# neuromodulation/PyPARRM

Hardware: NVIDIA B200
Metric: filter_data channel-samples/sec (higher is better)
Workload: dtype f64

## Files before the change

### pyparrm_b200/csrc/filter_comb_e.cuh

```cuda
#pragma once

#ifdef __CUDACC_RTC__
typedef signed char int8_t;
typedef int int32_t;
typedef unsigned int uint32_t;
typedef long long int64_t;
typedef unsigned long long uint64_t;
typedef unsigned long long uintptr_t;
#else
#include <stdint.h>
#endif

#ifndef PE_D
#define PE_T double
#define PE_D 200
#define PE_NK 2
#define PE_M0 20
#define PE_M1 10
#define PE_NB0 7
#define PE_NB1 2
#define PE_OFF0 -1969, -1954, -1923, -1877, -1846, -1831, -1800
#define PE_OFF1 -1908, 108
#define PE_NPLUS 1
#define PE_PLUS -2000
#define PE_NMINUS 0
#define PE_MINUS 0
#define PE_CENTRE -1
#define PE_U 10
#define PE_PF 2
#define PE_NTAPS 160
#define PE_WLO -2000
#define PE_WHI 2000
#define PE_BACK 108
#define PE_FWD 2000
#define PE_CTAS 2
#endif
#ifndef PE_VARIANT
#define PE_VARIANT 0
#endif

namespace parrm_e {

typedef PE_T T;
typedef double T2;
constexpr int D = PE_D;
constexpr int NK = PE_NK;
constexpr int M0 = PE_M0;
constexpr int M1 = PE_M1;
constexpr int NB0 = PE_NB0;
constexpr int NB1 = PE_NB1;
constexpr int NPLUS = PE_NPLUS;
constexpr int NMINUS = PE_NMINUS;
constexpr int CENTRE = PE_CENTRE;
constexpr int U = PE_U;
constexpr int PF = PE_PF;
constexpr int NTAPS = PE_NTAPS;
constexpr int WLO = PE_WLO;
constexpr int WHI = PE_WHI;
constexpr int BACK = PE_BACK;
constexpr int FWD = PE_FWD;
constexpr int ES = int(sizeof(T));
constexpr int VEC = 16 / ES;
constexpr int CH = U * D;
constexpr int HB = (BACK + CH - 1) / CH;
constexpr int HF = (FWD + CH - 1) / CH;
constexpr int MIR = HB + HF;
constexpr int Q = HB + HF + 1 + PF;
constexpr int GPB = (M0 + U - 1) / U;
constexpr int B = GPB * U;
constexpr int NPG = GPB;
constexpr int NW = (D + 31) / 32;
constexpr int NT = NW * 32 + 32;
constexpr int BAR_BYTES = ((2 * Q * 8 + 127) / 128) * 128;
constexpr int SMEM_BYTES = BAR_BYTES + (Q + MIR) * CH * ES;
static_assert((CH * ES) % 16 == 0, "chunk must be a whole number of 16-byte units");
static_assert(M0 >= M1 && M0 >= 1, "box lengths ordered");

__host__ __device__ constexpr int off0(int b) {
  constexpr int t[NB0 > 0 ? NB0 : 1] = {PE_OFF0};
  return t[b];
}
__host__ __device__ constexpr int off1(int b) {
  constexpr int t[NB1 > 0 ? NB1 : 1] = {PE_OFF1};
  return t[b];
}
__host__ __device__ constexpr int plus_tap(int i) {
  constexpr int t[NPLUS > 0 ? NPLUS : 1] = {PE_PLUS};
  return t[i];
}
__host__ __device__ constexpr int minus_tap(int i) {
  constexpr int t[NMINUS > 0 ? NMINUS : 1] = {PE_MINUS};
  return t[i];
}

struct Args {
  const T* x;
  T* out;
  const int32_t* taps;
  const int32_t* count;
  const T2* recip;
  int64_t ld_x, x_t0, n_x;
  int64_t ld_out, t0, n_out;
  int64_t n_total;
  int64_t total_groups;
  int32_t groups_per_chan;
  int32_t edge_start;
  int32_t edge_total;
  int32_t pad;
  unsigned long long* timeline;
  T neg_inv_n;
  T t_max;
};

__device__ __forceinline__ uint32_t smem_u32(const void* p) {
  return static_cast<uint32_t>(__cvta_generic_to_shared(p));
}
__device__ __forceinline__ void mbar_init(uint64_t* bar, uint32_t count) {
  asm volatile("mbarrier.init.shared::cta.b64 [%0], %1;" ::"r"(smem_u32(bar)), "r"(count));
}
__device__ __forceinline__ void mbar_expect_tx(uint64_t* bar, uint32_t bytes) {
  asm volatile("mbarrier.arrive.expect_tx.shared::cta.b64 _, [%0], %1;" ::"r"(smem_u32(bar)),
               "r"(bytes)
               : "memory");
}
__device__ __forceinline__ void mbar_arrive(uint64_t* bar) {
  asm volatile("mbarrier.arrive.shared::cta.b64 _, [%0];" ::"r"(smem_u32(bar)) : "memory");
}
__device__ __forceinline__ void mbar_wait(uint32_t bar, uint32_t parity) {
  asm volatile(
      "{\n"
      ".reg .pred p;\n"
      "WAIT_%=:\n"
      "mbarrier.try_wait.parity.shared::cta.b64 p, [%0], %1;\n"
      "@p bra DONE_%=;\n"
      "bra WAIT_%=;\n"
      "DONE_%=:\n"
      "}\n" ::"r"(bar),
      "r"(parity)
      : "memory");
}
__device__ __forceinline__ void bulk_g2s(void* dst_smem, const void* src_gmem, uint32_t bytes,
                                         uint64_t* bar) {
  asm volatile(
      "cp.async.bulk.shared::cluster.global.mbarrier::complete_tx::bytes [%0], [%1], %2, [%3];" ::
          "r"(smem_u32(dst_smem)),
      "l"(src_gmem), "r"(bytes), "r"(smem_u32(bar))
      : "memory");
}

__device__ __forceinline__ int64_t floor_div(int64_t a, int64_t b) {
  int64_t q = a / b;
  return (a % b != 0 && ((a < 0) != (b < 0))) ? q - 1 : q;
}
__device__ __forceinline__ int64_t min64(int64_t a, int64_t b) { return a < b ? a : b; }
__device__ __forceinline__ int64_t max64(int64_t a, int64_t b) { return a > b ? a : b; }

__device__ __forceinline__ T edge_value(const int32_t* __restrict__ count,
                                        const T2* __restrict__ recip, int64_t t, int64_t n_total,
                                        T xc, T tot) {
  const int64_t v1 = min64(max64(t, WLO - 1), WHI);
  const int64_t v2 = min64(max64(t - n_total, WLO - 1), WHI);
  const int n_in = count[v1 - (WLO - 1)] - count[v2 - (WLO - 1)];
  T y = xc - tot * T(recip[n_in]);
  if (n_in == 0) y = T(0);
  return y;
}

__device__ __noinline__ T direct_value(const int32_t* __restrict__ taps,
                                       const T2* __restrict__ recip, int64_t n_total, T t_max,
                                       const T* __restrict__ xrow, int64_t t, int64_t lo_valid,
                                       int64_t hi_valid) {
  T acc = T(0);
  int n_in = 0;
  for (int k = 0; k < NTAPS; ++k) {
    const int64_t g = t - taps[k];
    if (g < 0 || g >= n_total) continue;
    ++n_in;
    if (g >= lo_valid && g < hi_valid) acc += xrow[g];
  }
  if (n_in == 0) return T(0);
  const T y = xrow[t] - acc * T(recip[n_in]);
  return fabs(y) <= t_max ? y : T(0);
}

struct Walk {
  int pb;
  int rslot;
  int fslot;
  uint32_t fphase;
};

__device__ __forceinline__ void group_begin(Walk& w, uint32_t bars) {
  mbar_wait(bars + w.fslot * 8, w.fphase);
  if (++w.fslot == Q) {
    w.fslot = 0;
    w.fphase ^= 1u;
  }
}
__device__ __forceinline__ void group_end(Walk& w, uint32_t bars, int lane, unsigned wmask) {
  __syncwarp(wmask);
  if (lane == 0) {
    asm volatile("mbarrier.arrive.shared::cta.b64 _, [%0];" ::"r"(bars + (Q + w.rslot) * 8)
                 : "memory");
  }
  w.pb += CH * ES;
  if (++w.rslot == Q) {
    w.rslot = 0;
    w.pb -= Q * CH * ES;
  }
}

struct Rings {
  T r0[B];
  T r1[NK > 1 ? B : 1];
  T S0, S1;
};

__device__ __forceinline__ T ring_sum0(const Rings& r, int s) {
  T a = r.r0[s];
#pragma unroll
  for (int i = 1; i < M0; ++i) a += r.r0[(s + B - i) % B];
  return a;
}
__device__ __forceinline__ T ring_sum1(const Rings& r, int s) {
  if (NK < 2) return T(0);
  T a = r.r1[s];
#pragma unroll
  for (int i = 1; i < M1; ++i) a += r.r1[(s + B - i) % B];
  return a;
}

template <bool FAST>
__device__ __forceinline__ int run_block(Rings& r, Walk& w, const Args& a,
                                         const unsigned char* const smem, uint32_t bars,
                                         int lane, unsigned wmask, int c, T* const orow,
                                         int& bad_lo, int& bad_hi, int64_t Tb, int g,
                                         int n_groups) {
  const T neg_inv_n = a.neg_inv_n;
  const T t_max = a.t_max;
  T* const op = orow + Tb + c;
  int done = 0;
#pragma unroll
  for (int gi = 0; gi < GPB; ++gi) {
    if (!FAST && g + gi >= n_groups) break;
    group_begin(w, bars);
    int mode = 1;
    if (!FAST) {
      const int64_t Tn = Tb + int64_t(gi) * CH;
      const bool interior = (Tn - WHI >= 0) && (Tn + CH - WLO <= a.n_total);
      const bool all_out = (Tn >= a.t0) && (Tn + CH <= a.t0 + a.n_out);
      mode = (g + gi < NPG) ? 0 : ((interior && all_out) ? 1 : 2);
    }
    const unsigned char* const p = smem + w.pb;
#pragma unroll
    for (int js = 0; js < U; ++js) {
      const int s = gi * U + js;
      auto ld = [&](int off) {
        return *reinterpret_cast<const T*>(p + (HB * CH + js * D - off) * ES);
      };
      r.S0 -= r.r0[(s + B - M0) % B];
      if (NK > 1) r.S1 -= r.r1[(s + B - M1) % B];
      T e0 = ld(off0(0));
      if (NB0 > 1) {
        T e0b = ld(off0(1));
#pragma unroll
        for (int b = 2; b < NB0; ++b) {
          if (b & 1) e0b += ld(off0(b)); else e0 += ld(off0(b));
        }
        e0 += e0b;
      }
      r.r0[s] = e0;
      r.S0 += e0;
      T tot = r.S0;
      if (NK > 1) {
        T e1 = ld(off1(0));
        if (NB1 > 1) {
          T e1b = ld(off1(1));
#pragma unroll
          for (int b = 2; b < NB1; ++b) {
            if (b & 1) e1b += ld(off1(b)); else e1 += ld(off1(b));
          }
          e1 += e1b;
        }
        r.r1[s] = e1;
        r.S1 += e1;
        tot += r.S1;
      }
      T single = T(0);
      if (NPLUS > 0) {
        single = ld(plus_tap(0));
#pragma unroll
        for (int i = 1; i < NPLUS; ++i) single += ld(plus_tap(i));
      }
#pragma unroll
      for (int i = 0; i < NMINUS; ++i) single -= ld(minus_tap(i));
      const T xc = ld(0);
      if (CENTRE != 0) single = fma(T(CENTRE), xc, single);
      if (NPLUS > 0 || NMINUS > 0 || CENTRE != 0) tot += single;
      if (FAST) {
        T y = fma(tot, neg_inv_n, xc);
        if (__builtin_expect(!(fabs(y) <= t_max), 0)) {
          r.S0 = ring_sum0(r, s);
          r.S1 = ring_sum1(r, s);
          bad_lo = min(bad_lo, g * U + s);
          bad_hi = max(bad_hi, g * U + s);
          y = T(0);
        }
        op[s * D] = y;
      } else if (mode != 0) {
        const int64_t t = Tb + c + int64_t(s) * D;
        if (ES == 4 && mode == 2) {
          r.S0 = ring_sum0(r, s);
          r.S1 = ring_sum1(r, s);
          tot = r.S0;
          if (NK > 1) tot += r.S1;
          if (NPLUS > 0 || NMINUS > 0 || CENTRE != 0) tot += single;
        }
        T y = mode == 1 ? fma(tot, neg_inv_n, xc) : edge_value(a.count, a.recip, t, a.n_total, xc, tot);
        if (__builtin_expect(!(fabs(y) <= t_max), 0)) {
          r.S0 = ring_sum0(r, s);
          r.S1 = ring_sum1(r, s);
          bad_lo = min(bad_lo, g * U + s);
          bad_hi = max(bad_hi, g * U + s);
          y = T(0);
        }
        if (t >= a.t0 && t < a.t0 + a.n_out) op[s * D] = y;
      }
    }
    group_end(w, bars, lane, wmask);
    ++done;
  }
  return done;
}

extern "C" __global__ void __launch_bounds__(NT, PE_CTAS) parrm_filter_comb_e(const Args a) {
  extern __shared__ __align__(128) unsigned char smem_raw[];
  uint64_t* const full = reinterpret_cast<uint64_t*>(smem_raw);
  uint64_t* const empty = full + Q;
  T* const ring = reinterpret_cast<T*>(smem_raw + BAR_BYTES);
  const int tid = threadIdx.x;
  const int lane = tid & 31;
  const bool is_producer = tid >= NW * 32;

  if (tid == 0) {
    for (int s = 0; s < Q; ++s) {
      mbar_init(&full[s], 1);
      mbar_init(&empty[s], NW);
    }
    asm volatile("fence.mbarrier_init.release.cluster;" ::: "memory");
  }
  __syncthreads();

  const int64_t lo_valid = max64(0, a.x_t0);
  const int64_t hi_valid = min64(a.n_total, a.x_t0 + a.n_x);
#if PE_VARIANT & 2
  unsigned long long tl_start = 0, tl_pieces = 0;
  if (tid == 0) asm volatile("mov.u64 %0, %%globaltimer;" : "=l"(tl_start));
#endif
  const int gpc = a.groups_per_chan;
  const int vpc = gpc + a.edge_total;
  const int64_t G_begin = a.total_groups * int64_t(blockIdx.x) / int64_t(gridDim.x);
  const int64_t G_end = a.total_groups * int64_t(blockIdx.x + 1) / int64_t(gridDim.x);
  const uint32_t bars = smem_u32(smem_raw);

  int fslot = 0;
  uint32_t fphase = 0;
  int rslot = 0;

  for (int64_t G = G_begin; G < G_end;) {
    const int64_t chan = G / vpc;
    const int v0 = int(G - chan * vpc);
    const int v1 = int(min64(vpc, v0 + (G_end - G)));
    G += v1 - v0;
    const int s0 = min(max(v0 - a.edge_start, 0), gpc);
    const int s1 = min(max(v1 - a.edge_start, 0), gpc);
    if (s1 <= s0) continue;
    const T* const xrow = a.x + chan * a.ld_x - a.x_t0;
    T* const orow = a.out + chan * a.ld_out - a.t0;
    const int gamma = int((VEC - int((reinterpret_cast<uintptr_t>(xrow) / ES) % VEC)) % VEC);
    const int64_t j_first = floor_div(a.t0 - gamma, CH);
    const int64_t j_last = floor_div(a.t0 + a.n_out - 1 - gamma, CH);
    const int64_t n_first = j_first + s0;
    const int64_t n_end = min64(j_first + s1, j_last + 1);
    if (n_first >= n_end) continue;
#if PE_VARIANT & 2
    ++tl_pieces;
#endif
    const int n_groups = NPG + int(n_end - n_first);
    const int n_chunks = n_groups + HB + HF;
    const int64_t c_first = n_first - NPG - HB;

    if (is_producer) {
      for (int i = 0; i < n_chunks; ++i) {
        const int64_t g0 = gamma + (c_first + i) * int64_t(CH);
        T* const dst = ring + fslot * CH;
        mbar_wait(bars + (Q + fslot) * 8, fphase ^ 1u);
        if (g0 >= lo_valid && g0 + CH <= hi_valid) {
          if (lane == 0) {
            asm volatile("fence.proxy.async.shared::cta;" ::: "memory");
            const bool mirror = fslot < MIR;
            mbar_expect_tx(&full[fslot], uint32_t(CH * ES) * (mirror ? 2u : 1u));
            bulk_g2s(dst, xrow + g0, uint32_t(CH * ES), &full[fslot]);
            if (mirror) bulk_g2s(dst + Q * CH, xrow + g0, uint32_t(CH * ES), &full[fslot]);
          }
        } else {
          for (int e = lane; e < CH; e += 32) {
            const int64_t g = g0 + e;
            const T v = (g >= lo_valid && g < hi_valid) ? xrow[g] : T(0);
            dst[e] = v;
            if (fslot < MIR) dst[Q * CH + e] = v;
          }
          __syncwarp();
          if (lane == 0) mbar_arrive(&full[fslot]);
        }
        if (++fslot == Q) {
          fslot = 0;
          fphase ^= 1u;
        }
      }
      continue;
    }

    if (tid >= D) continue;
    const int c = tid;
    const unsigned wmask = (tid | 31) < D ? 0xffffffffu : ((1u << (D & 31)) - 1u);
    for (int i = 0; i < HB + HF; ++i) {
      mbar_wait(bars + fslot * 8, fphase);
      if (++fslot == Q) {
        fslot = 0;
        fphase ^= 1u;
      }
    }
    Rings r;
#pragma unroll
    for (int s = 0; s < B; ++s) r.r0[s] = T(0);
#pragma unroll
    for (int s = 0; s < (NK > 1 ? B : 1); ++s) r.r1[s] = T(0);
    const int64_t T0 = gamma + (n_first - NPG) * int64_t(CH);
    Walk w;
    w.pb = BAR_BYTES + (rslot * CH + c) * ES;
    w.rslot = rslot;
    w.fslot = fslot;
    w.fphase = fphase;
    int bad_lo = 1 << 30, bad_hi = -1;
    for (int g = 0; g < n_groups;) {
      const int64_t Tb = T0 + int64_t(g) * CH;
      r.S0 = ring_sum0(r, B - 1);
      r.S1 = ring_sum1(r, B - 1);
      const bool fast = g >= NPG && g + GPB <= n_groups && Tb - WHI >= 0 &&
                        Tb + int64_t(B) * D - WLO <= a.n_total && Tb >= a.t0 &&
                        Tb + int64_t(B) * D <= a.t0 + a.n_out;
      if (fast) {
        g += run_block<true>(r, w, a, smem_raw, bars, lane, wmask, c, orow, bad_lo, bad_hi,
                             Tb, g, n_groups);
      } else {
        g += run_block<false>(r, w, a, smem_raw, bars, lane, wmask, c, orow, bad_lo, bad_hi,
                              Tb, g, n_groups);
      }
    }
    rslot = w.rslot;
    fslot = w.fslot;
    fphase = w.fphase;
    for (int k = bad_lo; k <= bad_hi; ++k) {
      const int64_t t = T0 + c + int64_t(k) * D;
      if (t >= a.t0 && t < a.t0 + a.n_out)
        orow[t] = direct_value(a.taps, a.recip, a.n_total, a.t_max, xrow, t, lo_valid, hi_valid);
    }
    __syncwarp(wmask);
    for (int i = 0; i < HB + HF; ++i) {
      if (lane == 0) mbar_arrive(&empty[rslot]);
      if (++rslot == Q) rslot = 0;
    }
  }
#if PE_VARIANT & 2
  if (tid == 0 && a.timeline) {
    unsigned long long tl_end;
    unsigned smid;
    asm volatile("mov.u64 %0, %%globaltimer;" : "=l"(tl_end));
    asm volatile("mov.u32 %0, %%smid;" : "=r"(smid));
    a.timeline[4 * blockIdx.x + 0] = smid;
    a.timeline[4 * blockIdx.x + 1] = tl_start;
    a.timeline[4 * blockIdx.x + 2] = tl_end;
    a.timeline[4 * blockIdx.x + 3] = tl_pieces;
  }
#endif
}

}
```

### pyparrm_b200/csrc/filter_jit.cu

```cuda
#include <cuda.h>
#include <dlfcn.h>
#include <string.h>

#include <algorithm>
#include <map>
#include <mutex>
#include <string>
#include <vector>

#include "common.cuh"
#include "filter_jit.h"
#include "filter_plan.h"

namespace parrm {
namespace {

const char kCombESource[] =
#include "filter_comb_e_src.inc"
    ;

typedef struct _nvrtcProgram* nvrtcProgram;
struct Nvrtc {
  void* handle = nullptr;
  int (*CreateProgram)(nvrtcProgram*, const char*, const char*, int, const char* const*,
                       const char* const*) = nullptr;
  int (*CompileProgram)(nvrtcProgram, int, const char* const*) = nullptr;
  int (*GetCUBINSize)(nvrtcProgram, size_t*) = nullptr;
  int (*GetCUBIN)(nvrtcProgram, char*) = nullptr;
  int (*GetProgramLogSize)(nvrtcProgram, size_t*) = nullptr;
  int (*GetProgramLog)(nvrtcProgram, char*) = nullptr;
  int (*DestroyProgram)(nvrtcProgram*) = nullptr;
  const char* (*GetErrorString)(int) = nullptr;
  bool ok = false;
};

Nvrtc* nvrtc() {
  static Nvrtc n;
  static std::once_flag once;
  std::call_once(once, [] {
    const char* names[] = {"libnvrtc.so.12", "libnvrtc.so", "/usr/local/cuda/lib64/libnvrtc.so.12",
                           "/usr/local/cuda/lib64/libnvrtc.so"};
    for (const char* name : names) {
      n.handle = dlopen(name, RTLD_NOW | RTLD_LOCAL);
      if (n.handle) break;
    }
    if (!n.handle) return;
#define PARRM_NVRTC_SYM(field, sym)                                             \
  n.field = reinterpret_cast<decltype(n.field)>(dlsym(n.handle, sym));          \
  if (!n.field) return;
    PARRM_NVRTC_SYM(CreateProgram, "nvrtcCreateProgram")
    PARRM_NVRTC_SYM(CompileProgram, "nvrtcCompileProgram")
    PARRM_NVRTC_SYM(GetCUBINSize, "nvrtcGetCUBINSize")
    PARRM_NVRTC_SYM(GetCUBIN, "nvrtcGetCUBIN")
    PARRM_NVRTC_SYM(GetProgramLogSize, "nvrtcGetProgramLogSize")
    PARRM_NVRTC_SYM(GetProgramLog, "nvrtcGetProgramLog")
    PARRM_NVRTC_SYM(DestroyProgram, "nvrtcDestroyProgram")
    PARRM_NVRTC_SYM(GetErrorString, "nvrtcGetErrorString")
#undef PARRM_NVRTC_SYM
    n.ok = true;
  });
  return &n;
}

struct Driver {
  CUresult (*ModuleLoadData)(CUmodule*, const void*) = nullptr;
  CUresult (*ModuleGetFunction)(CUfunction*, CUmodule, const char*) = nullptr;
  CUresult (*FuncSetAttribute)(CUfunction, CUfunction_attribute, int) = nullptr;
  CUresult (*FuncGetAttribute)(int*, CUfunction_attribute, CUfunction) = nullptr;
  CUresult (*LaunchKernel)(CUfunction, unsigned, unsigned, unsigned, unsigned, unsigned, unsigned,
                           unsigned, CUstream, void**, void**) = nullptr;
  CUresult (*GetErrorString)(CUresult, const char**) = nullptr;
  bool ok = false;
};

Driver* driver() {
  static Driver d;
  static std::once_flag once;
  std::call_once(once, [] {
    auto get = [](const char* name, void** fn) {
      cudaDriverEntryPointQueryResult st;
      return cudaGetDriverEntryPoint(name, fn, cudaEnableDefault, &st) == cudaSuccess &&
             st == cudaDriverEntryPointSuccess && *fn != nullptr;
    };
    d.ok = get("cuModuleLoadData", reinterpret_cast<void**>(&d.ModuleLoadData)) &&
           get("cuModuleGetFunction", reinterpret_cast<void**>(&d.ModuleGetFunction)) &&
           get("cuFuncSetAttribute", reinterpret_cast<void**>(&d.FuncSetAttribute)) &&
           get("cuFuncGetAttribute", reinterpret_cast<void**>(&d.FuncGetAttribute)) &&
           get("cuLaunchKernel", reinterpret_cast<void**>(&d.LaunchKernel)) &&
           get("cuGetErrorString", reinterpret_cast<void**>(&d.GetErrorString));
  });
  return &d;
}

int driver_fail(CUresult rc, const char* what) {
  const char* msg = nullptr;
  if (driver()->GetErrorString) driver()->GetErrorString(rc, &msg);
  set_error("%s: %s", what, msg ? msg : "driver error");
  return PARRM_ERR_CUDA;
}

struct Kernel {
  CUfunction fn = nullptr;
  int smem_bytes = 0, threads = 0, regs = 0, ctas_per_sm = 1;
  int chunk = 0, priming_groups = 0;
};

std::mutex g_mutex;
std::map<std::string, Kernel> g_cache;

std::string join(const int32_t* v, int n) {
  std::string s;
  for (int i = 0; i < n; ++i) {
    if (i) s += ",";
    s += std::to_string(v[i]);
  }
  if (n == 0) s = "0";
  return s;
}

}

bool comb_e_shape(const FilterPlanHeader* hdr, const int32_t* terms, int dtype,
                  const FilterTuning* tune, CombEShape* out) {
  const FilterPlanHeader* sec = hdr;
  if (hdr->kind != kPlanComb || sec->n_kinds < 1 || sec->n_kinds > 2) return false;
  CombEShape s;
  memset(&s, 0, sizeof(s));
  s.es = dtype == PARRM_F64 ? 8 : 4;
  s.d = sec->stride;
  s.nk = sec->n_kinds;
  const int nb[2] = {sec->n_box[0], sec->n_kinds > 1 ? sec->n_box[1] : 0};
  int first = 0;
  if (s.nk == 2 && sec->window[1] > sec->window[0]) first = 1;
  const int32_t* box[2] = {terms, terms + nb[0]};
  s.m[0] = sec->window[first];
  s.nb[0] = nb[first];
  s.off[0] = box[first];
  if (s.nk == 2) {
    s.m[1] = sec->window[1 - first];
    s.nb[1] = nb[1 - first];
    s.off[1] = box[1 - first];
  } else {
    s.m[1] = 1;
    s.nb[1] = 0;
    s.off[1] = nullptr;
  }
  s.n_plus = sec->n_plus;
  s.n_minus = sec->n_minus;
  s.plus = terms + nb[0] + nb[1];
  s.minus = s.plus + s.n_plus;
  s.centre = sec->centre;
  s.n_taps = hdr->n_taps;
  s.w_lo = hdr->w_min < 0 ? hdr->w_min : 0;
  s.w_hi = hdr->w_max > 0 ? hdr->w_max : 0;
  int lo = 0, hi = 0;
  const int n_all = nb[0] + nb[1] + s.n_plus + s.n_minus;
  for (int i = 0; i < n_all; ++i) {
    lo = terms[i] < lo ? terms[i] : lo;
    hi = terms[i] > hi ? terms[i] : hi;
  }
  s.back = hi;
  s.fwd = -lo;
  if (s.d < kPatternFirstMinStride || s.d > kPatternFirstMaxStride) return false;
  if (n_all > 96 || s.nb[0] < 1) return false;
  const int ring_regs = (s.m[0] + (s.nk > 1 ? s.m[1] : 0)) * (s.es / 4);
  const int threads = pattern_first_threads(s.d);
  auto reg_budget = [&](int ctas) { return pattern_first_reg_budget(s.d, ctas); };
  if (ring_regs + kPatternFirstStepRegs > reg_budget(1)) return false;
  int ctas_first = ring_regs + kPatternFirstStepRegs <= reg_budget(2) ? 2 : 1;
  if (s.es == 4 && 3 * threads <= 2048 && ring_regs + 40 <= reg_budget(3)) ctas_first = 3;
  if (tune && tune->ctas_per_sm > 0) ctas_first = tune->ctas_per_sm;
  const int pf_max = (tune && tune->prefetch_chunks > 0) ? tune->prefetch_chunks : 2;
  const int pf_min = std::min(pf_max, 2);
  auto smem_for = [&](int u, int pf) {
    const int64_t ch = int64_t(u) * s.d;
    const int64_t hb = (s.back + ch - 1) / ch, hf = (s.fwd + ch - 1) / ch;
    const int64_t q = hb + hf + 1 + pf;
    return ((2 * q * 8 + 127) / 128) * 128 + (q + hb + hf) * ch * s.es;
  };
  auto usable = [&](int u) {
    return u >= 1 && (int64_t(u) * s.d * s.es) % 16 == 0 && (s.m[0] + u - 1) / u * u <= 64;
  };
  for (int ctas = ctas_first; ctas >= 1; --ctas) {
    const int64_t budget = int64_t(227) * 1024 / ctas - 1024;
    int u = 0;
    if (tune && tune->steps_per_chunk > 0) {
      u = tune->steps_per_chunk;
      if (!usable(u) || smem_for(u, pf_min) > budget) u = 0;
    } else {
      for (int cand = s.m[0]; cand >= 1 && u == 0; --cand)
        if (s.m[0] % cand == 0 && int64_t(cand) * s.d * s.es <= 32768 &&
            int64_t(cand) * s.d >= 512 && usable(cand) && smem_for(cand, pf_min) <= budget)
          u = cand;
      const int u_hi = int(std::max<int64_t>(1, 20480 / (int64_t(s.d) * s.es)));
      for (int cand = u_hi; cand >= 1 && u == 0; --cand)
        if (usable(cand) && smem_for(cand, pf_min) <= budget) u = cand;
      for (int cand = 1; cand <= 64 && u == 0; ++cand)
        if (usable(cand) && smem_for(cand, pf_min) <= budget) u = cand;
    }
    if (u == 0) continue;
    int pf = pf_min;
    while (pf < pf_max && smem_for(u, pf + 1) <= budget) ++pf;
    s.smem_bytes = int(smem_for(u, pf));
    s.ctas = ctas;
    s.u = u;
    s.pf = pf;
    s.variant = tune ? tune->variant : 0;
    *out = s;
    return true;
  }
  return false;
}

static int compile_cubin(const CombEShape& s, std::vector<char>* cubin) {
  Nvrtc* n = nvrtc();
  if (!n->ok) {
    const char* why = dlerror();
    set_error("parrm filter: NVRTC (libnvrtc.so.12) could not be opened: %s", why ? why : "?");
    return PARRM_ERR_UNSUPPORTED;
  }
  std::vector<std::string> opts = {
      "--gpu-architecture=sm_100a", "-std=c++17", "-lineinfo",
      std::string("-DPE_T=") + (s.es == 8 ? "double" : "float"),
      "-DPE_D=" + std::to_string(s.d), "-DPE_NK=" + std::to_string(s.nk),
      "-DPE_M0=" + std::to_string(s.m[0]), "-DPE_M1=" + std::to_string(s.m[1]),
      "-DPE_NB0=" + std::to_string(s.nb[0]), "-DPE_NB1=" + std::to_string(s.nb[1]),
      "-DPE_OFF0=" + join(s.off[0], s.nb[0]), "-DPE_OFF1=" + join(s.off[1], s.nb[1]),
      "-DPE_NPLUS=" + std::to_string(s.n_plus), "-DPE_PLUS=" + join(s.plus, s.n_plus),
      "-DPE_NMINUS=" + std::to_string(s.n_minus), "-DPE_MINUS=" + join(s.minus, s.n_minus),
      "-DPE_CENTRE=" + std::to_string(s.centre), "-DPE_U=" + std::to_string(s.u),
      "-DPE_PF=" + std::to_string(s.pf), "-DPE_NTAPS=" + std::to_string(s.n_taps),
      "-DPE_WLO=" + std::to_string(s.w_lo), "-DPE_WHI=" + std::to_string(s.w_hi),
      "-DPE_BACK=" + std::to_string(s.back), "-DPE_FWD=" + std::to_string(s.fwd),
      "-DPE_CTAS=" + std::to_string(s.ctas), "-DPE_VARIANT=" + std::to_string(s.variant)};
  std::vector<const char*> copts;
  for (const std::string& o : opts) copts.push_back(o.c_str());
  nvrtcProgram prog = nullptr;
  int rc = n->CreateProgram(&prog, kCombESource, "filter_comb_e.cu", 0, nullptr, nullptr);
  if (rc != 0) {
    set_error("nvrtcCreateProgram: %s", n->GetErrorString(rc));
    return PARRM_ERR_CUDA;
  }
  rc = n->CompileProgram(prog, int(copts.size()), copts.data());
  if (rc != 0) {
    size_t log_size = 0;
    n->GetProgramLogSize(prog, &log_size);
    std::string log(log_size + 1, '\0');
    if (log_size) n->GetProgramLog(prog, &log[0]);
    set_error("nvrtcCompileProgram: %s\n%.380s", n->GetErrorString(rc), log.c_str());
    n->DestroyProgram(&prog);
    return PARRM_ERR_CUDA;
  }
  size_t cubin_size = 0;
  n->GetCUBINSize(prog, &cubin_size);
  cubin->resize(cubin_size);
  rc = n->GetCUBIN(prog, cubin->data());
  n->DestroyProgram(&prog);
  if (rc != 0 || cubin_size == 0) {
    set_error("nvrtcGetCUBIN: %s", n->GetErrorString(rc));
    return PARRM_ERR_CUDA;
  }
  return PARRM_OK;
}

int comb_e_compile_only(const CombEShape& s, size_t* cubin_bytes) {
  std::vector<char> cubin;
  const int rc = compile_cubin(s, &cubin);
  if (rc == PARRM_OK && cubin_bytes) *cubin_bytes = cubin.size();
  return rc;
}

static int build_kernel(const CombEShape& s, Kernel* out) {
  Driver* d = driver();
  if (!d->ok) {
    set_error("parrm filter: CUDA driver entry points unavailable");
    return PARRM_ERR_UNSUPPORTED;
  }
  std::vector<char> cubin;
  const int rc = compile_cubin(s, &cubin);
  if (rc != PARRM_OK) return rc;
  PARRM_CUDA_OK(cudaFree(nullptr));
  CUmodule mod = nullptr;
  CUresult cr = d->ModuleLoadData(&mod, cubin.data());
  if (cr != CUDA_SUCCESS) return driver_fail(cr, "cuModuleLoadData");
  Kernel k;
  cr = d->ModuleGetFunction(&k.fn, mod, "parrm_filter_comb_e");
  if (cr != CUDA_SUCCESS) return driver_fail(cr, "cuModuleGetFunction");
  k.smem_bytes = s.smem_bytes;
  k.threads = ((s.d + 31) / 32) * 32 + 32;
  k.ctas_per_sm = s.ctas;
  k.chunk = s.u * s.d;
  k.priming_groups = (s.m[0] + s.u - 1) / s.u;
  cr = d->FuncSetAttribute(k.fn, CU_FUNC_ATTRIBUTE_MAX_DYNAMIC_SHARED_SIZE_BYTES, k.smem_bytes);
  if (cr != CUDA_SUCCESS) return driver_fail(cr, "cuFuncSetAttribute(max dynamic shared memory)");
  d->FuncSetAttribute(k.fn, CU_FUNC_ATTRIBUTE_PREFERRED_SHARED_MEMORY_CARVEOUT, 100);
  d->FuncGetAttribute(&k.regs, CU_FUNC_ATTRIBUTE_NUM_REGS, k.fn);
  *out = k;
  return PARRM_OK;
}

bool comb_e_cached(const CombEShape& s) {
  int dev = 0;
  if (cudaGetDevice(&dev) != cudaSuccess) return false;
  const std::string key = comb_e_key(s, dev);
  std::lock_guard<std::mutex> lock(g_mutex);
  return g_cache.count(key) != 0;
}

std::string comb_e_key(const CombEShape& s, int dev) {
  std::string key = std::to_string(dev) + "|" + std::to_string(s.es) + "|" + std::to_string(s.d) +
                    "|" + std::to_string(s.nk) + "|" + std::to_string(s.m[0]) + "|" +
                    std::to_string(s.m[1]) + "|" + join(s.off[0], s.nb[0]) + "|" +
                    join(s.off[1], s.nb[1]) + "|" + join(s.plus, s.n_plus) + "|" +
                    join(s.minus, s.n_minus) + "|" + std::to_string(s.centre) + "|" +
                    std::to_string(s.u) + "|" + std::to_string(s.pf) + "|" +
                    std::to_string(s.n_taps) + "|" + std::to_string(s.w_lo) + "|" +
                    std::to_string(s.w_hi) + "|" + std::to_string(s.ctas) + "|" +
                    std::to_string(s.variant);
  return key;
}

int launch_comb_e(const CombEShape& s, const void* d_x, void* d_out, const int32_t* d_taps,
                  const int32_t* d_count, const double* d_recip,
                  int64_t ld_x, int64_t x_t0, int64_t n_x, int64_t ld_out, int64_t t0,
                  int64_t n_out, int64_t n_total, int64_t n_chans, cudaStream_t stream,
                  int* regs_out, unsigned long long timeline) {
  int dev = 0;
  PARRM_CUDA_OK(cudaGetDevice(&dev));
  const std::string key = comb_e_key(s, dev);
  Kernel k;
  {
    std::lock_guard<std::mutex> lock(g_mutex);
    auto it = g_cache.find(key);
    if (it == g_cache.end()) {
      const int rc = build_kernel(s, &k);
      if (rc != PARRM_OK) return rc;
      g_cache[key] = k;
    } else {
      k = it->second;
    }
  }
  if (regs_out) *regs_out = k.regs;
  struct Args {
    const void* x;
    void* out;
    const int32_t* taps;
    const int32_t* count;
    const double* recip;
    int64_t ld_x, x_t0, n_x, ld_out, t0, n_out, n_total, total_groups;
    int32_t groups_per_chan, edge_start, edge_total, pad;
    unsigned long long timeline;
    unsigned char consts[16];
  } a;
  a.x = d_x; a.out = d_out; a.taps = d_taps; a.count = d_count; a.recip = d_recip;
  a.ld_x = ld_x; a.x_t0 = x_t0; a.n_x = n_x;
  a.ld_out = ld_out; a.t0 = t0; a.n_out = n_out; a.n_total = n_total;
  const int64_t ch = k.chunk;
  a.groups_per_chan = int32_t(ceil_div(n_out + ch - 1, ch));
  const int gpb = k.priming_groups;
  const int edge_end = 2 * gpb;
  a.edge_start = s.variant & 4 ? 0 : 2 * gpb + 2 + edge_end;
  a.edge_total = s.variant & 4 ? 0 : a.edge_start + edge_end;
  a.total_groups = n_chans * int64_t(a.groups_per_chan + a.edge_total);
  a.pad = 0;
  a.timeline = timeline;
  memset(a.consts, 0, sizeof(a.consts));
  if (s.es == 8) {
    const double v[2] = {-1.0 / double(s.n_taps), 1.7976931348623157e308};
    memcpy(a.consts, v, sizeof(v));
  } else {
    const float v[2] = {-1.0f / float(s.n_taps), 3.402823466e38f};
    memcpy(a.consts, v, sizeof(v));
  }
  const int64_t resident = int64_t(kNumSMs) * k.ctas_per_sm;
  const int64_t min_groups = int64_t(4) * k.priming_groups;
  const int64_t grid =
      max64(1, min64(resident, n_chans * int64_t(a.groups_per_chan) / min_groups));
  void* params[] = {&a};
  const CUresult cr = driver()->LaunchKernel(k.fn, unsigned(grid), 1, 1, unsigned(k.threads), 1, 1,
                                             unsigned(k.smem_bytes), stream, params, nullptr);
  if (cr != CUDA_SUCCESS) return driver_fail(cr, "cuLaunchKernel(parrm_filter_comb_e)");
  return PARRM_OK;
}

}
```

### pyparrm_b200/csrc/filter_jit.h

```cpp
#pragma once
#include <cuda_runtime.h>
#include <stdint.h>

#include <string>

#include "filter_plan.h"

namespace parrm {

struct FilterTuning {
  int kernel;
  int steps_per_chunk;
  int prefetch_chunks;
  int ctas_per_sm;
  int variant;
  unsigned long long timeline;
};

struct CombEShape {
  int es;
  int d, nk, m[2], nb[2];
  const int32_t* off[2];
  int n_plus, n_minus;
  const int32_t *plus, *minus;
  int centre, n_taps, w_lo, w_hi, back, fwd;
  int u, pf, ctas, smem_bytes, variant;
};

bool comb_e_shape(const FilterPlanHeader* hdr, const int32_t* terms, int dtype,
                  const FilterTuning* tune, CombEShape* out);
std::string comb_e_key(const CombEShape& s, int dev);
bool comb_e_cached(const CombEShape& s);
int comb_e_compile_only(const CombEShape& s, size_t* cubin_bytes);
int launch_comb_e(const CombEShape& s, const void* d_x, void* d_out, const int32_t* d_taps,
                  const int32_t* d_count, const double* d_recip,
                  int64_t ld_x, int64_t x_t0, int64_t n_x, int64_t ld_out, int64_t t0,
                  int64_t n_out, int64_t n_total, int64_t n_chans, cudaStream_t stream,
                  int* regs_out, unsigned long long timeline = 0);

}
```

Baseline: 309.5 billion.

## Keep f64 running-sum rings in tensor memory and add a register delay line

Moves the per-thread float64 box-sum ring buffers from registers into Blackwell tensor memory (tcgen05 alloc/ld/st), prefetching the slot to subtract one batch ahead. It also adds a register delay line that reuses a lead tap's value for other taps lagging it by multiples of D, so those taps skip shared-memory loads. The aim is to cut register pressure and shared-memory load traffic. In exchange it adds tensor-memory load/store waits on the critical path, requires full warps (dead lanes now run with masked work), and resums the rings through tensor memory on outliers.

```diff
diff --git a/profiles/r3/ab_tmem.py b/profiles/r3/ab_tmem.py
--- /dev/null
+++ b/profiles/r3/ab_tmem.py
@@ -0,0 +1,78 @@
+
+import json
+import os
+import subprocess
+import sys
+
+WORKER = r"""
+import hashlib, json, sys
+root = sys.argv[1]
+sys.path.insert(0, root)
+import numpy as np, torch
+from oracle import parrm_oracle as oracle
+from pyparrm_b200 import _native as K
+from pyparrm_b200._engine import get_engine
+eng = get_engine()
+def taps_of(fs, fa, hw, d):
+    p = fs / fa * (1 + 3e-6)
+    return oracle.tap_offsets(p, p / 50, hw, 0, d)
+cases = [("cfg2", taps_of(2000, 130, 2000, "both"), 64, 1_200_000),
+         ("cfg3", taps_of(1000, 145, 2469, "both"), 256, 3_600_000),
+         ("cfg4", taps_of(30000, 130, 2311, "past"), 384, 3_000_000),
+         ("cfg1", oracle.tap_offsets(1.3311148014466094, 0.01, 2000, 20, "both"), 64, 1_200_000)]
+res = {}
+for name, taps, c, n in cases:
+    g = torch.Generator(device="cuda").manual_seed(5)
+    d_x = torch.randn((c, n), dtype=torch.float64, device="cuda", generator=g)
+    d_y = torch.empty_like(d_x)
+    for _ in range(3):
+        eng.filter_device(d_x, taps, d_out=d_y, kernel=K.KERNEL_SPECIALISED)
+    torch.cuda.synchronize()
+    e0, e1 = torch.cuda.Event(enable_timing=True), torch.cuda.Event(enable_timing=True)
+    reps = 40 if c * n < 1e8 else 10
+    e0.record()
+    for _ in range(reps):
+        eng.filter_device(d_x, taps, d_out=d_y, kernel=K.KERNEL_SPECIALISED)
+    e1.record()
+    torch.cuda.synchronize()
+    res[name] = {"ms": e0.elapsed_time(e1) / reps, "kernel": eng.last_filter_kernel}
+    if name == "cfg2":
+        res[name]["sha256"] = hashlib.sha256(d_y.cpu().numpy().tobytes()).hexdigest()
+    del d_x, d_y
+print(json.dumps(res))
+"""
+
+
+def main():
+    args = [a for a in sys.argv[1:] if not a.startswith("--")]
+    reps = int(sys.argv[sys.argv.index("--reps") + 1]) if "--reps" in sys.argv else 3
+    if "--reps" in sys.argv:
+        args.remove(str(reps))
+    here = os.path.dirname(os.path.dirname(os.path.dirname(os.path.abspath(__file__))))
+    builds = {"parent": os.path.abspath(args[0]),
+              "branch": os.path.abspath(args[1]) if len(args) > 1 else here}
+    smi = subprocess.run(["nvidia-smi", "--query-gpu=name,power.limit,clocks.max.sm",
+                          "--format=csv,noheader"], capture_output=True, text=True).stdout
+    print("gpu:", smi.strip().splitlines()[0] if smi.strip() else "?", flush=True)
+    runs = {name: [] for name in builds}
+    for rep in range(reps):
+        for name, root in builds.items():
+            out = subprocess.run([sys.executable, "-c", WORKER, root], capture_output=True,
+                                 text=True, check=True).stdout.strip().splitlines()[-1]
+            runs[name].append(json.loads(out))
+            print(rep, name, out, flush=True)
+    print("summary (ms per pass: median, spread of repeats, branch / parent):")
+    for case in runs["parent"][0]:
+        med = {}
+        for name in builds:
+            v = sorted(r[case]["ms"] for r in runs[name])
+            med[name] = v[len(v) // 2]
+            print(f"  {case} {name}: {med[name]:.4f} ms, spread {v[-1] - v[0]:.4f} ms", flush=True)
+        print(f"  {case} branch / parent = {med['branch'] / med['parent']:.4f}")
+    digests = {name: {r["cfg2"]["sha256"] for r in runs[name]} for name in builds}
+    print("cfg2 outputs identical:", digests["parent"] == digests["branch"]
+          and len(digests["parent"]) == 1)
+
+
+if __name__ == "__main__":
+    main()
diff --git a/pyparrm_b200/csrc/filter_comb_e.cuh b/pyparrm_b200/csrc/filter_comb_e.cuh
--- a/pyparrm_b200/csrc/filter_comb_e.cuh
+++ b/pyparrm_b200/csrc/filter_comb_e.cuh
@@ -37,6 +37,13 @@
 #endif
 #ifndef PE_VARIANT
 #define PE_VARIANT 0
+#endif
+#ifndef PE_TMB
+#define PE_TMB 0
+#endif
+#ifndef PE_LINE
+#define PE_LINE 0
+#define PE_LEAD 0
 #endif
 
 namespace parrm_e {
@@ -93,6 +100,33 @@
   return t[i];
 }
 
+constexpr int LINE = PE_LINE;
+constexpr int LEAD = PE_LEAD;
+constexpr int LSLOTS = LINE > 0 ? LINE : 1;
+static_assert(LINE == 0 || (B % LINE == 0 && LINE <= B), "delay line slots must be static");
+__host__ __device__ constexpr int line_lag(int off) {
+  return (LINE > 0 && off > LEAD && (off - LEAD) % D == 0 && (off - LEAD) / D <= LINE)
+             ? (off - LEAD) / D
+             : 0;
+}
+
+constexpr bool TM = PE_TMB > 0;
+constexpr int TMB = TM ? PE_TMB : 1;
+constexpr int CV = ES / 4;
+constexpr int NQ = (NW + 3) / 4;
+constexpr int TM_C1 = CV * M0;
+constexpr int TM_VALS = M0 + (NK > 1 ? M1 : 0);
+constexpr int TM_NEED = NQ * TM_VALS * CV;
+constexpr int TM_COLS = TM_NEED <= 32 ? 32 : TM_NEED <= 64 ? 64 : TM_NEED <= 128 ? 128
+                        : TM_NEED <= 256 ? 256 : 512;
+constexpr int TMQ = TM ? NK * TMB * CV : 1;
+static_assert(!TM || ES == 8, "tensor-memory rings: float64 only");
+static_assert(!TM || (B % M0 == 0 && (NK < 2 || B % M1 == 0)), "one ring turn per block");
+static_assert(!TM || (M0 % TMB == 0 && (NK < 2 || M1 % TMB == 0)), "a batch is contiguous slots");
+static_assert(!TM || 2 * TMB <= (NK > 1 ? M1 : M0), "a batch is requested one batch ahead");
+static_assert(!TM || (B / TMB) % 2 == 0, "buffer parity static across blocks");
+static_assert(!TM || TM_COLS * PE_CTAS <= 512, "rings do not fit tensor memory");
+
 struct Args {
   const T* x;
   T* out;
@@ -148,6 +182,55 @@
       : "memory");
 }
 
+template <int N>
+__device__ __forceinline__ void tm_ld(uint32_t ta, uint32_t* r) {
+  if constexpr (N >= 16) {
+    asm volatile(
+        "tcgen05.ld.sync.aligned.32x32b.x16.b32 {%0, %1, %2, %3, %4, %5, %6, %7, %8, %9, %10, "
+        "%11, %12, %13, %14, %15}, [%16];"
+        : "=r"(r[0]), "=r"(r[1]), "=r"(r[2]), "=r"(r[3]), "=r"(r[4]), "=r"(r[5]), "=r"(r[6]),
+          "=r"(r[7]), "=r"(r[8]), "=r"(r[9]), "=r"(r[10]), "=r"(r[11]), "=r"(r[12]),
+          "=r"(r[13]), "=r"(r[14]), "=r"(r[15])
+        : "r"(ta));
+    tm_ld<N - 16>(ta + 16, r + 16);
+  } else if constexpr (N >= 8) {
+    asm volatile(
+        "tcgen05.ld.sync.aligned.32x32b.x8.b32 {%0, %1, %2, %3, %4, %5, %6, %7}, [%8];"
+        : "=r"(r[0]), "=r"(r[1]), "=r"(r[2]), "=r"(r[3]), "=r"(r[4]), "=r"(r[5]), "=r"(r[6]),
+          "=r"(r[7])
+        : "r"(ta));
+    tm_ld<N - 8>(ta + 8, r + 8);
+  } else if constexpr (N >= 4) {
+    asm volatile("tcgen05.ld.sync.aligned.32x32b.x4.b32 {%0, %1, %2, %3}, [%4];"
+                 : "=r"(r[0]), "=r"(r[1]), "=r"(r[2]), "=r"(r[3])
+                 : "r"(ta));
+    tm_ld<N - 4>(ta + 4, r + 4);
+  } else if constexpr (N >= 2) {
+    asm volatile("tcgen05.ld.sync.aligned.32x32b.x2.b32 {%0, %1}, [%2];"
+                 : "=r"(r[0]), "=r"(r[1])
+                 : "r"(ta));
+    tm_ld<N - 2>(ta + 2, r + 2);
+  } else if constexpr (N == 1) {
+    asm volatile("tcgen05.ld.sync.aligned.32x32b.x1.b32 {%0}, [%1];" : "=r"(r[0]) : "r"(ta));
+  }
+}
+template <int N>
+__device__ __forceinline__ void tm_wait_ld(uint32_t* r) {
+  asm volatile("tcgen05.wait::ld.sync.aligned;" ::: "memory");
+#pragma unroll
+  for (int i = 0; i < N; ++i) asm volatile("" : "+r"(r[i]));
+}
+__device__ __forceinline__ void tm_wait_st() {
+  asm volatile("tcgen05.wait::st.sync.aligned;" ::: "memory");
+}
+__device__ __forceinline__ void tm_st(uint32_t ta, double v) {
+  asm volatile("tcgen05.st.sync.aligned.32x32b.x2.b32 [%0], {%1, %2};" ::"r"(ta),
+               "r"(uint32_t(__double2loint(v))), "r"(uint32_t(__double2hiint(v))));
+}
+__device__ __forceinline__ double tm_value(const uint32_t* r) {
+  return __hiloint2double(int(r[1]), int(r[0]));
+}
+
 __device__ __forceinline__ int64_t floor_div(int64_t a, int64_t b) {
   int64_t q = a / b;
   return (a % b != 0 && ((a < 0) != (b < 0))) ? q - 1 : q;
@@ -211,31 +294,84 @@
 }
 
 struct Rings {
-  T r0[B];
-  T r1[NK > 1 ? B : 1];
+  T r0[TM ? 1 : B];
+  T r1[(NK > 1 && !TM) ? B : 1];
   T S0, S1;
+  T line[LSLOTS];
+  uint32_t ta;
+  uint32_t q[2][TMQ];
 };
 
 __device__ __forceinline__ T ring_sum0(const Rings& r, int s) {
-  T a = r.r0[s];
-#pragma unroll
-  for (int i = 1; i < M0; ++i) a += r.r0[(s + B - i) % B];
+  T a = r.r0[TM ? 0 : s];
+#pragma unroll
+  for (int i = 1; i < M0; ++i) a += r.r0[TM ? 0 : (s + B - i) % B];
   return a;
 }
 __device__ __forceinline__ T ring_sum1(const Rings& r, int s) {
   if (NK < 2) return T(0);
-  T a = r.r1[s];
-#pragma unroll
-  for (int i = 1; i < M1; ++i) a += r.r1[(s + B - i) % B];
+  T a = r.r1[TM ? 0 : s];
+#pragma unroll
+  for (int i = 1; i < M1; ++i) a += r.r1[TM ? 0 : (s + B - i) % B];
   return a;
 }
 
-template <bool FAST>
+__device__ __forceinline__ void tm_request(Rings& r, int s) {
+  uint32_t* const q = r.q[(s / TMB) % 2];
+  tm_ld<TMB * CV>(r.ta + CV * (s % M0), q);
+  if (NK > 1) tm_ld<TMB * CV>(r.ta + TM_C1 + CV * (s % M1), q + TMB * CV);
+}
+__device__ __forceinline__ void tm_block_sums(Rings& r) {
+  tm_wait_st();
+  {
+    uint32_t v[CV * M0];
+    tm_ld<CV * M0>(r.ta, v);
+    tm_wait_ld<CV * M0>(v);
+    T a = T(tm_value(v + CV * ((B - 1) % M0)));
+#pragma unroll
+    for (int i = 1; i < M0; ++i) a += T(tm_value(v + CV * ((B - 1 - i) % M0)));
+    r.S0 = a;
+  }
+  if (NK > 1) {
+    uint32_t v[CV * (NK > 1 ? M1 : 1)];
+    tm_ld<CV * (NK > 1 ? M1 : 1)>(r.ta + TM_C1, v);
+    tm_wait_ld<CV * (NK > 1 ? M1 : 1)>(v);
+    T a = T(tm_value(v + CV * ((B - 1) % M1)));
+#pragma unroll
+    for (int i = 1; i < M1; ++i) a += T(tm_value(v + CV * ((B - 1 - i) % M1)));
+    r.S1 = a;
+  } else {
+    r.S1 = T(0);
+  }
+}
+__device__ __forceinline__ void tm_resum(Rings& r, int s, bool need) {
+  tm_wait_st();
+  T a[2] = {T(0), T(0)};
+#pragma unroll
+  for (int k = 0; k < NK; ++k) {
+    const int m = k ? M1 : M0;
+    const uint32_t base = r.ta + (k ? TM_C1 : 0);
+#pragma unroll 1
+    for (int i = 0; i < m; ++i) {
+      uint32_t v[CV];
+      tm_ld<CV>(base + CV * ((s + B - i) % m), v);
+      tm_wait_ld<CV>(v);
+      a[k] = i ? a[k] + T(tm_value(v)) : T(tm_value(v));
+    }
+  }
+  if (need) {
+    r.S0 = a[0];
+    r.S1 = a[1];
+  }
+}
+
+template <bool FAST, bool PART>
 __device__ __forceinline__ int run_block(Rings& r, Walk& w, const Args& a,
                                          const unsigned char* const smem, uint32_t bars,
-                                         int lane, unsigned wmask, int c, T* const orow,
-                                         int& bad_lo, int& bad_hi, int64_t Tb, int g,
-                                         int n_groups) {
+                                         int lane, unsigned wmask, bool live_lane, int c,
+                                         T* const orow, int& bad_lo, int& bad_hi, int64_t Tb,
+                                         int g, int n_groups) {
+  const bool live = PART ? live_lane : true;
   const T neg_inv_n = a.neg_inv_n;
   const T t_max = a.t_max;
   T* const op = orow + Tb + c;
@@ -255,11 +391,30 @@
 #pragma unroll
     for (int js = 0; js < U; ++js) {
       const int s = gi * U + js;
+      auto lds = [&](int off) {
+        T v = T(0);
+        if (live) v = *reinterpret_cast<const T*>(p + (HB * CH + js * D - off) * ES);
+        return v;
+      };
+      const T lead = LINE > 0 ? lds(LEAD) : T(0);
       auto ld = [&](int off) {
-        return *reinterpret_cast<const T*>(p + (HB * CH + js * D - off) * ES);
+        if (FAST && line_lag(off) > 0) return r.line[(s + B - line_lag(off)) % LSLOTS];
+        if (LINE > 0 && off == LEAD) return lead;
+        return lds(off);
       };
-      r.S0 -= r.r0[(s + B - M0) % B];
-      if (NK > 1) r.S1 -= r.r1[(s + B - M1) % B];
+      if constexpr (TM) {
+        const uint32_t* const q = r.q[(s / TMB) % 2];
+        if (s % TMB == 0) {
+          tm_wait_ld<TMQ>(r.q[(s / TMB) % 2]);
+          tm_wait_st();
+          tm_request(r, (s + TMB) % B);
+        }
+        r.S0 -= T(tm_value(q + CV * (s % TMB)));
+        if (NK > 1) r.S1 -= T(tm_value(q + TMB * CV + CV * (s % TMB)));
+      } else {
+        r.S0 -= r.r0[(s + B - M0) % B];
+        if (NK > 1) r.S1 -= r.r1[(s + B - M1) % B];
+      }
       T e0 = ld(off0(0));
       if (NB0 > 1) {
         T e0b = ld(off0(1));
@@ -269,7 +424,7 @@
         }
         e0 += e0b;
       }
-      r.r0[s] = e0;
+      if constexpr (TM) tm_st(r.ta + CV * (s % M0), e0); else r.r0[s] = e0;
       r.S0 += e0;
       T tot = r.S0;
       if (NK > 1) {
@@ -282,7 +437,7 @@
           }
           e1 += e1b;
         }
-        r.r1[s] = e1;
+        if constexpr (TM) tm_st(r.ta + TM_C1 + CV * (s % M1), e1); else r.r1[s] = e1;
         r.S1 += e1;
         tot += r.S1;
       }
@@ -299,14 +454,18 @@
       if (NPLUS > 0 || NMINUS > 0 || CENTRE != 0) tot += single;
       if (FAST) {
         T y = fma(tot, neg_inv_n, xc);
-        if (__builtin_expect(!(fabs(y) <= t_max), 0)) {
-          r.S0 = ring_sum0(r, s);
-          r.S1 = ring_sum1(r, s);
+        const bool bad = live && !(fabs(y) <= t_max);
+        if (__builtin_expect(bad, 0)) {
+          if (!TM) {
+            r.S0 = ring_sum0(r, s);
+            r.S1 = ring_sum1(r, s);
+          }
           bad_lo = min(bad_lo, g * U + s);
           bad_hi = max(bad_hi, g * U + s);
           y = T(0);
         }
-        op[s * D] = y;
+        if (TM && __builtin_expect(__any_sync(0xffffffffu, bad), 0)) tm_resum(r, s, bad);
+        if (live) op[s * D] = y;
       } else if (mode != 0) {
         const int64_t t = Tb + c + int64_t(s) * D;
         if (ES == 4 && mode == 2) {
@@ -317,15 +476,20 @@
           if (NPLUS > 0 || NMINUS > 0 || CENTRE != 0) tot += single;
         }
         T y = mode == 1 ? fma(tot, neg_inv_n, xc) : edge_value(a.count, a.recip, t, a.n_total, xc, tot);
-        if (__builtin_expect(!(fabs(y) <= t_max), 0)) {
-          r.S0 = ring_sum0(r, s);
-          r.S1 = ring_sum1(r, s);
+        const bool bad = live && !(fabs(y) <= t_max);
+        if (__builtin_expect(bad, 0)) {
+          if (!TM) {
+            r.S0 = ring_sum0(r, s);
+            r.S1 = ring_sum1(r, s);
+          }
           bad_lo = min(bad_lo, g * U + s);
           bad_hi = max(bad_hi, g * U + s);
           y = T(0);
         }
-        if (t >= a.t0 && t < a.t0 + a.n_out) op[s * D] = y;
-      }
+        if (TM && __builtin_expect(__any_sync(0xffffffffu, bad), 0)) tm_resum(r, s, bad);
+        if (live && t >= a.t0 && t < a.t0 + a.n_out) op[s * D] = y;
+      }
+      if constexpr (LINE > 0) r.line[s % LSLOTS] = lead;
     }
     group_end(w, bars, lane, wmask);
     ++done;
@@ -349,7 +513,17 @@
     }
     asm volatile("fence.mbarrier_init.release.cluster;" ::: "memory");
   }
+  __shared__ uint32_t tmem_slot;
+  if (TM && tid < 32) {
+    asm volatile("tcgen05.alloc.cta_group::1.sync.aligned.shared::cta.b32 [%0], %1;" ::"r"(
+                     smem_u32(&tmem_slot)),
+                 "n"(TM_COLS));
+    asm volatile("tcgen05.relinquish_alloc_permit.cta_group::1.sync.aligned;");
+  }
+  if (TM) asm volatile("tcgen05.fence::before_thread_sync;");
   __syncthreads();
+  if (TM) asm volatile("tcgen05.fence::after_thread_sync;");
+  const uint32_t tmem_base = TM ? tmem_slot : 0u;
 
   const int64_t lo_valid = max64(0, a.x_t0);
   const int64_t hi_valid = min64(a.n_total, a.x_t0 + a.n_x);
@@ -421,9 +595,10 @@
       continue;
     }
 
-    if (tid >= D) continue;
+    if (!TM && tid >= D) continue;
+    const bool live = !TM || tid < D;
     const int c = tid;
-    const unsigned wmask = (tid | 31) < D ? 0xffffffffu : ((1u << (D & 31)) - 1u);
+    const unsigned wmask = (TM || (tid | 31) < D) ? 0xffffffffu : ((1u << (D & 31)) - 1u);
     for (int i = 0; i < HB + HF; ++i) {
       mbar_wait(bars + fslot * 8, fphase);
       if (++fslot == Q) {
@@ -433,9 +608,16 @@
     }
     Rings r;
 #pragma unroll
-    for (int s = 0; s < B; ++s) r.r0[s] = T(0);
-#pragma unroll
-    for (int s = 0; s < (NK > 1 ? B : 1); ++s) r.r1[s] = T(0);
+    for (int s = 0; s < (TM ? 1 : B); ++s) r.r0[s] = T(0);
+#pragma unroll
+    for (int s = 0; s < ((NK > 1 && !TM) ? B : 1); ++s) r.r1[s] = T(0);
+#pragma unroll
+    for (int s = 0; s < LSLOTS; ++s) r.line[s] = T(0);
+    if constexpr (TM) {
+      const int warp = __shfl_sync(0xffffffffu, tid >> 5, 0);
+      r.ta = tmem_base + (uint32_t((warp & 3) * 32) << 16) + uint32_t((warp >> 2) * CV * TM_VALS);
+      tm_request(r, 0);
+    }
     const int64_t T0 = gamma + (n_first - NPG) * int64_t(CH);
     Walk w;
     w.pb = BAR_BYTES + (rslot * CH + c) * ES;
@@ -445,23 +627,35 @@
     int bad_lo = 1 << 30, bad_hi = -1;
     for (int g = 0; g < n_groups;) {
       const int64_t Tb = T0 + int64_t(g) * CH;
-      r.S0 = ring_sum0(r, B - 1);
-      r.S1 = ring_sum1(r, B - 1);
+      if constexpr (TM) {
+        tm_block_sums(r);
+      } else {
+        r.S0 = ring_sum0(r, B - 1);
+        r.S1 = ring_sum1(r, B - 1);
+      }
       const bool fast = g >= NPG && g + GPB <= n_groups && Tb - WHI >= 0 &&
                         Tb + int64_t(B) * D - WLO <= a.n_total && Tb >= a.t0 &&
                         Tb + int64_t(B) * D <= a.t0 + a.n_out;
-      if (fast) {
-        g += run_block<true>(r, w, a, smem_raw, bars, lane, wmask, c, orow, bad_lo, bad_hi,
-                             Tb, g, n_groups);
+      if (fast && !(TM && (tid | 31) >= D)) {
+        g += run_block<true, false>(r, w, a, smem_raw, bars, lane, wmask, live, c, orow, bad_lo,
+                                    bad_hi, Tb, g, n_groups);
+      } else if (fast) {
+        g += run_block<true, TM>(r, w, a, smem_raw, bars, lane, wmask, live, c, orow, bad_lo,
+                                 bad_hi, Tb, g, n_groups);
       } else {
-        g += run_block<false>(r, w, a, smem_raw, bars, lane, wmask, c, orow, bad_lo, bad_hi,
-                              Tb, g, n_groups);
-      }
+        g += run_block<false, TM>(r, w, a, smem_raw, bars, lane, wmask, live, c, orow, bad_lo,
+                                  bad_hi, Tb, g, n_groups);
+      }
+    }
+    if constexpr (TM) {
+      tm_wait_ld<TMQ>(r.q[0]);
+      tm_wait_st();
     }
     rslot = w.rslot;
     fslot = w.fslot;
     fphase = w.fphase;
     for (int k = bad_lo; k <= bad_hi; ++k) {
+      if (!live) break;
       const int64_t t = T0 + c + int64_t(k) * D;
       if (t >= a.t0 && t < a.t0 + a.n_out)
         orow[t] = direct_value(a.taps, a.recip, a.n_total, a.t_max, xrow, t, lo_valid, hi_valid);
@@ -471,6 +665,13 @@
       if (lane == 0) mbar_arrive(&empty[rslot]);
       if (++rslot == Q) rslot = 0;
     }
+  }
+  if (TM) {
+    asm volatile("tcgen05.fence::before_thread_sync;");
+    __syncthreads();
+    if (tid < 32)
+      asm volatile("tcgen05.dealloc.cta_group::1.sync.aligned.b32 %0, %1;" ::"r"(tmem_base),
+                   "n"(TM_COLS));
   }
 #if PE_VARIANT & 2
   if (tid == 0 && a.timeline) {
diff --git a/pyparrm_b200/csrc/filter_jit.cu b/pyparrm_b200/csrc/filter_jit.cu
--- a/pyparrm_b200/csrc/filter_jit.cu
+++ b/pyparrm_b200/csrc/filter_jit.cu
@@ -116,6 +116,53 @@
   }
   if (n == 0) s = "0";
   return s;
+}
+
+void choose_tmem_form(CombEShape* s, int ring_regs) {
+  s->tmb = 0;
+  s->line = 0;
+  s->lead = 0;
+  if (s->es != 8 || (s->variant & 8)) return;
+  const int b_steps = (s->m[0] + s->u - 1) / s->u * s->u;
+  const int m_min = s->nk > 1 ? s->m[1] : s->m[0];
+  if (b_steps % s->m[0] != 0 || b_steps % m_min != 0) return;
+  int tmb = 0;
+  for (int b = 1; b <= 2; ++b)
+    if (s->m[0] % b == 0 && m_min % b == 0 && 2 * b <= m_min && (b_steps / b) % 2 == 0) tmb = b;
+  if (tmb == 0) return;
+  const int nq = ((s->d + 31) / 32 + 3) / 4;
+  const int need = nq * 2 * (s->m[0] + (s->nk > 1 ? s->m[1] : 0));
+  int cols = 32;
+  while (cols < need) cols *= 2;
+  if (cols * s->ctas > 512) return;
+  std::vector<int> terms;
+  for (int k = 0; k < s->nk; ++k) terms.insert(terms.end(), s->off[k], s->off[k] + s->nb[k]);
+  terms.insert(terms.end(), s->plus, s->plus + s->n_plus);
+  terms.insert(terms.end(), s->minus, s->minus + s->n_minus);
+  terms.push_back(0);
+  const int line_budget = ring_regs - 2 * 2 * s->nk * tmb;
+  int best_served = 0;
+  for (int lead : terms) {
+    for (int len = 1; len <= b_steps && 2 * len <= line_budget; ++len) {
+      if (b_steps % len != 0) continue;
+      CombEShape t = *s;
+      t.line = len;
+      t.lead = lead;
+      int served = 0;
+      bool is_lead = true;
+      for (int off : terms) {
+        if (off < lead && (lead - off) % s->d == 0) is_lead = false;
+        served += comb_e_line_serves(t, off) ? 1 : 0;
+      }
+      if (is_lead && served > best_served) {
+        best_served = served;
+        s->line = len;
+        s->lead = lead;
+      }
+    }
+  }
+  if (best_served == 0) return;
+  s->tmb = tmb;
 }
 
 }
@@ -206,6 +253,7 @@
     s.u = u;
     s.pf = pf;
     s.variant = tune ? tune->variant : 0;
+    choose_tmem_form(&s, ring_regs);
     *out = s;
     return true;
   }
@@ -232,7 +280,9 @@
       "-DPE_PF=" + std::to_string(s.pf), "-DPE_NTAPS=" + std::to_string(s.n_taps),
       "-DPE_WLO=" + std::to_string(s.w_lo), "-DPE_WHI=" + std::to_string(s.w_hi),
       "-DPE_BACK=" + std::to_string(s.back), "-DPE_FWD=" + std::to_string(s.fwd),
-      "-DPE_CTAS=" + std::to_string(s.ctas), "-DPE_VARIANT=" + std::to_string(s.variant)};
+      "-DPE_CTAS=" + std::to_string(s.ctas), "-DPE_VARIANT=" + std::to_string(s.variant),
+      "-DPE_TMB=" + std::to_string(s.tmb), "-DPE_LINE=" + std::to_string(s.line),
+      "-DPE_LEAD=" + std::to_string(s.lead)};
   std::vector<const char*> copts;
   for (const std::string& o : opts) copts.push_back(o.c_str());
   nvrtcProgram prog = nullptr;
@@ -316,7 +366,8 @@
                     std::to_string(s.u) + "|" + std::to_string(s.pf) + "|" +
                     std::to_string(s.n_taps) + "|" + std::to_string(s.w_lo) + "|" +
                     std::to_string(s.w_hi) + "|" + std::to_string(s.ctas) + "|" +
-                    std::to_string(s.variant);
+                    std::to_string(s.variant) + "|" + std::to_string(s.tmb) + "|" +
+                    std::to_string(s.line) + "|" + std::to_string(s.lead);
   return key;
 }
 
diff --git a/pyparrm_b200/csrc/filter_jit.h b/pyparrm_b200/csrc/filter_jit.h
--- a/pyparrm_b200/csrc/filter_jit.h
+++ b/pyparrm_b200/csrc/filter_jit.h
@@ -25,7 +25,13 @@
   const int32_t *plus, *minus;
   int centre, n_taps, w_lo, w_hi, back, fwd;
   int u, pf, ctas, smem_bytes, variant;
+  int tmb;
+  int line, lead;
 };
+
+inline bool comb_e_line_serves(const CombEShape& s, int off) {
+  return s.line > 0 && off > s.lead && (off - s.lead) % s.d == 0 && (off - s.lead) / s.d <= s.line;
+}
 
 bool comb_e_shape(const FilterPlanHeader* hdr, const int32_t* terms, int dtype,
                   const FilterTuning* tune, CombEShape* out);
```

Measured after the change: 189.9 billion (median of 6 runs). -38.6%, worse.
